# oscka/rag-llm-k8s

Measured on AMD Instinct MI355X. Metric: end-to-end RAG query p50 latency + gen tokens/sec, Llama-3.1-8B top-k=4, higher is better.
Workload: dtype bf16; 1 GPU; model=Llama-3.1-8B-Instruct, embedder=all-MiniLM-L6-v2, index=FlatL2 10000 vectors (HBM-resident; 10000 embedded chunks), retrieve_k=4, context_k=4, global_batch=32, seq_len=5198, parallelism=dp1

## Files before the change

### csrc/kernels/gemm_w4.hip

```cpp
#include <stdlib.h>

#include <utility>

#include "common.h"
using namespace ragk;

namespace {

constexpr int WBM = 256, WBN = 256, WBK = 64;
constexpr int W4_THREADS = 256;
constexpr int W_TILE_A = WBM * WBK * 2;
constexpr int W_TILE_B = WBN * WBK * 2;
constexpr int W_BUF = W_TILE_A + W_TILE_B;
constexpr int W4_LDS = 2 * W_BUF;
constexpr int WGROUP_M = 8;
constexpr int W4_MIN_KT = 3;

__device__ __forceinline__ int wswz(int row, int chunk) { return chunk ^ ((row >> 1) & 7); }

template <typename F, int... Ms>
__device__ __forceinline__ void static_for_impl(F&& f, std::integer_sequence<int, Ms...>) {
  (f(std::integral_constant<int, Ms>{}), ...);
}
template <int N, typename F>
// ... 390 lines not shown

__device__ __forceinline__ void w4_read_f0(int g, const unsigned (&rbA)[2], const unsigned (&rbB)[2],
                                           bf16x8 (&a0)[8], bf16x8 (&b0)[8]) {
  const unsigned buf = (unsigned)(g & 1) * W_BUF;
  const unsigned rb0 = rbB[0] + buf, ra0 = rbA[0] + buf;
  static_for<8>([&](auto jc) __attribute__((always_inline)) {
    constexpr int j = decltype(jc)::value;
    h_read(b0[j], rb0, j * 2048);
  });
  static_for<8>([&](auto ic) __attribute__((always_inline)) {
    constexpr int i = decltype(ic)::value;
    h_read(a0[i], ra0, i * 2048);
  });
}

__device__ __forceinline__ void w4_origin(int tile, int nwg, int tiles_m, int tiles_n, int& m0, int& n0) {
  const int logical = xcd_remap(tile, nwg);
  const int group = logical / (WGROUP_M * tiles_n);
  const int first_m = group * WGROUP_M;
  const int gm = min(tiles_m - first_m, WGROUP_M);
  const int in_group = logical % (WGROUP_M * tiles_n);
  m0 = (first_m + in_group % gm) * WBM;
  n0 = (in_group / gm) * WBN;
}

template <int EPI, bool OUT_F32, bool KSPLIT = false>
__global__ __launch_bounds__(W4_THREADS, 1) void gemm_w4_kernel(const bf16_t* __restrict__ A, int lda,
                                                                const bf16_t* __restrict__ B, int ldb, void* C,
                                                                int ldc, const bf16_t* __restrict__ bias,
                                                                const bf16_t* resid, int ldr, int M, int N, int K,
                                                                int nsplit, RopeKV rk) {
  __shared__ __attribute__((aligned(16))) char smem[W4_LDS];
  const int tid = threadIdx.x, lane = tid & 63;
  const int wid = __builtin_amdgcn_readfirstlane(tid >> 6);
  const int wr = wid >> 1, wc = wid & 1;
  const int fr = lane & 15, fh = lane >> 4;
  const int tiles_m = (M + WBM - 1) / WBM, tiles_n = (N + WBN - 1) / WBN;
  const int nwg = tiles_m * tiles_n;
  const int nwt = KSPLIT ? nwg * nsplit : nwg;
  const int nk = K / WBK;
  const int Nout = EPI == EPI_SILU_MUL ? N / 2 : N;
  const i32x4 srd_a = make_srd(A, (unsigned)M * (unsigned)lda * 2u);
  const i32x4 srd_b = make_srd(B, (unsigned)N * (unsigned)ldb * 2u);

  constexpr int EV = w4_epi_vmem<EPI, OUT_F32>();
  constexpr int VMH0 = H_VM + EV > 63 ? 63 : H_VM + EV;
  constexpr bool LATE_F0 = !(EPI == EPI_NONE || EPI == EPI_SILU_MUL || (EPI == EPI_RESID && !OUT_F32));
  static_assert(EPI != EPI_ROPE_KV || (!OUT_F32 && !KSPLIT), "rope epilogue: bf16 output, no split-K");

  int tile = blockIdx.x;
  int z = KSPLIT ? tile / nwg : 0;
  int m0, n0;
  w4_origin(tile - z * nwg, nwg, tiles_m, tiles_n, m0, n0);
  int off_a[8], off_b[8];
  w4_offsets<false>(lda, m0, M, wid, lane, off_a);
  w4_offsets<true>(ldb, n0, N, wid, lane, off_b);
  if constexpr (KSPLIT) {
#pragma unroll
    for (int i = 0; i < 8; ++i) {
      off_a[i] += z * K * 2;
      off_b[i] += z * K * 2;
    }
  }
  w4_stage(srd_a, off_a, 0, smem, wid);
  w4_stage(srd_b, off_b, 0, smem + W_TILE_A, wid);
  w4_stage(srd_a, off_a, WBK, smem + W_BUF, wid);
  w4_stage(srd_b, off_b, WBK, smem + W_BUF + W_TILE_A, wid);
  __builtin_amdgcn_s_waitcnt(0x0F70);
// ... 14 lines not shown
    }
  }

  f32x4 acc[8][8];
  int g = 0;
  for (;;) {
    const int next = tile + (int)gridDim.x;
    const bool has_next = next < nwt;
    w4_iter_h<true, VMH0>(smem, g, srd_a, srd_b, off_a, off_b, 2, wid, rbA, rbB, acc, a0, b0, a1, b1);
    ++g;
    for (int t = 1; t + 2 < nk; ++t, ++g)
      w4_iter_h<false, H_VM>(smem, g, srd_a, srd_b, off_a, off_b, t + 2, wid, rbA, rbB, acc, a0, b0, a1, b1);
    int nm0, nn0;
    const int ntile = has_next ? next : tile;
    const int nz = KSPLIT ? ntile / nwg : 0;
    w4_origin(ntile - nz * nwg, nwg, tiles_m, tiles_n, nm0, nn0);
    {
      int ln;
      asm volatile("v_mbcnt_lo_u32_b32 %0, -1, 0\n\tv_mbcnt_hi_u32_b32 %0, -1, %0" : "=v"(ln));
      w4_offsets<false>(lda, nm0, M, wid, ln, off_a);
      w4_offsets<true>(ldb, nn0, N, wid, ln, off_b);
      if constexpr (KSPLIT) {
#pragma unroll
        for (int i = 0; i < 8; ++i) {
          off_a[i] += nz * K * 2;
          off_b[i] += nz * K * 2;
        }
      }
    }
    w4_iter_h<false, H_VM>(smem, g, srd_a, srd_b, off_a, off_b, 0, wid, rbA, rbB, acc, a0, b0, a1, b1);
    ++g;
// ... 32 lines not shown
  }
}

static int g_w4_grid = -1;
static int w4_grid(int nwg) {
  if (g_w4_grid < 0) {
    int cus = 0, dev = 0;
    if (hipGetDevice(&dev) != hipSuccess ||
        hipDeviceGetAttribute(&cus, hipDeviceAttributeMultiprocessorCount, dev) != hipSuccess)
      cus = 256;
    g_w4_grid = (cus / 8) * 8;
  }
  return (g_w4_grid == 0 || g_w4_grid >= nwg) ? nwg : g_w4_grid;
}

template <int EPI, bool F32>
int launch_w4(const void* A, int lda, const void* B, int ldb, void* C, int ldc, const void* bias, const void* resid,
              int ldr, int M, int N, int K, hipStream_t st) {
  const int nwg = ((M + WBM - 1) / WBM) * ((N + WBN - 1) / WBN);
  hipLaunchKernelGGL((gemm_w4_kernel<EPI, F32>), dim3(w4_grid(nwg)), dim3(W4_THREADS), 0, st, (const bf16_t*)A, lda,
                     (const bf16_t*)B, ldb, C, ldc, (const bf16_t*)bias, (const bf16_t*)resid, ldr, M, N, K, 1,
                     RopeKV{});
  return (int)hipGetLastError();
}

}

RAGK_API int ragk_gemm_w4_set_grid(int g) {
  g_w4_grid = g < 0 ? -1 : g;
  return 0;
}

RAGK_API int ragk_gemm_w4(const void* A, int lda, const void* B, int ldb, void* C, int ldc, const void* bias,
                          const void* resid, int ldr, int M, int N, int K, int epi, int out_f32, hipStream_t st) {
  if (M <= 0 || N <= 0 || K <= 0) return 0;
  if (K % WBK != 0 || K / WBK < W4_MIN_KT) return (int)hipErrorInvalidValue;
  const long long rows_b = (epi == EPI_SILU_MUL) ? 2LL * N : (long long)N;
  if ((long long)M * lda * 2 >= (1LL << 31) || rows_b * ldb * 2 >= (1LL << 31))
    return (int)hipErrorInvalidValue;
  if (epi == EPI_SILU_MUL) {
    if (N % 128 != 0 || out_f32) return (int)hipErrorInvalidValue;
    return launch_w4<EPI_SILU_MUL, false>(A, lda, B, ldb, C, ldc, bias, resid, ldr, M, 2 * N, K, st);
  }
  if (N % 8 != 0) return (int)hipErrorInvalidValue;
#define RAGK_W4_CASE(E) \
  case E:               \
    return out_f32 ? launch_w4<E, true>(A, lda, B, ldb, C, ldc, bias, resid, ldr, M, N, K, st) \
                   : launch_w4<E, false>(A, lda, B, ldb, C, ldc, bias, resid, ldr, M, N, K, st);
  switch (epi) {
    RAGK_W4_CASE(EPI_NONE)
    RAGK_W4_CASE(EPI_BIAS)
    RAGK_W4_CASE(EPI_RESID)
    RAGK_W4_CASE(EPI_BIAS_RESID)
    RAGK_W4_CASE(EPI_BIAS_GELU)
    RAGK_W4_CASE(EPI_GELU)
    RAGK_W4_CASE(EPI_BIAS_GELU_TANH)
    default:
      return (int)hipErrorInvalidValue;
  }
#undef RAGK_W4_CASE
}

RAGK_API int ragk_gemm_w4_splitk(const void* A, int lda, const void* B, int ldb, float* P, int M, int N, int K,
                                 int nsplit, hipStream_t st) {
  if (M <= 0 || N <= 0 || K <= 0) return 0;
  if (nsplit < 1 || K % nsplit || (K / nsplit) % WBK || (K / nsplit) / WBK < W4_MIN_KT || N % 8 || !P)
    return (int)hipErrorInvalidValue;
  if ((long long)M * lda * 2 >= (1LL << 31) || (long long)N * ldb * 2 >= (1LL << 31)) return (int)hipErrorInvalidValue;
  const int nwg = ((M + WBM - 1) / WBM) * ((N + WBN - 1) / WBN);
  hipLaunchKernelGGL((gemm_w4_kernel<EPI_NONE, true, true>), dim3(w4_grid(nwg * nsplit)), dim3(W4_THREADS), 0, st,
                     (const bf16_t*)A, lda, (const bf16_t*)B, ldb, (void*)P, N, nullptr, nullptr, 0, M, N, K / nsplit,
                     nsplit, RopeKV{});
  return (int)hipGetLastError();
}

RAGK_API int ragk_gemm_w4_rope_kv(const void* A, int lda, const void* B, int ldb, void* C, int ldc, int M, int K,
                                  const int* pos, const int* slot, const float* cos_t, const float* sin_t, void* kc,
                                  void* vc, int Hq, int Hkv, int BS, hipStream_t st) {
  if (M <= 0) return 0;
  const int N = (Hq + 2 * Hkv) * 128;
  if (K % WBK != 0 || K / WBK < W4_MIN_KT || Hq < 1 || Hkv < 1 || BS < 1 || N % WBN != 0) return (int)hipErrorInvalidValue;
  if (!pos || !slot || !cos_t || !sin_t || !kc || !vc || ldc % 8 != 0) return (int)hipErrorInvalidValue;
  if ((long long)M * lda * 2 >= (1LL << 31) || (long long)N * ldb * 2 >= (1LL << 31)) return (int)hipErrorInvalidValue;
  const int nwg = ((M + WBM - 1) / WBM) * (N / WBN);
  const RopeKV rk{pos, slot, cos_t, sin_t, (bf16_t*)kc, (bf16_t*)vc, Hq, Hkv, BS};
  hipLaunchKernelGGL((gemm_w4_kernel<EPI_ROPE_KV, false>), dim3(w4_grid(nwg)), dim3(W4_THREADS), 0, st,
                     (const bf16_t*)A, lda, (const bf16_t*)B, ldb, C, ldc, nullptr, nullptr, 0, M, N, K, 1, rk);
  return (int)hipGetLastError();
}
```

### rag_llm_k8s_amd/engine/llm_engine.py

```python
from __future__ import annotations

import itertools
import logging
import os
import threading
import time
from collections import deque
from dataclasses import dataclass, field
from typing import List, Optional

import numpy as np
import torch

from ..models.llama import StepInput
from ..ops.backend import AttnMeta
from ..ops.fp8 import kv_cache_dtype_name, kv_cache_torch_dtype
from ..utils import faults
from .kv_manager import BLOCK, make_block_manager

SMALL_BATCH_TOPK_MAX_B = 64
SMALL_BATCH_TOPK_CHUNK = 4096

log = logging.getLogger(__name__)

# ... 395 lines not shown
            p = np.arange(start, start + n, dtype=np.int32)
            if start + n <= len(s.prompt):
                ids.append(s.prompt_np[start:start + n])
            else:
                ids.append(np.asarray([s.token_at(i) for i in range(start, start + n)], dtype=np.int32))
            pos.append(p)
            slots.append(table[p // BLOCK] * BLOCK + p % BLOCK)
            cu.append(cu[-1] + n)
            kvl.append(start + n)
            qlens.append(n)
            nb = min(len(table), self.max_blocks)
            bts[ci, :nb] = table[:nb]
            if start + n == len(s.prompt) or (start + n == s.length and start >= len(s.prompt)):
                out_rows.append(cu[-1] - 1)
                out_seqs.append(s)
        from ..ops.native import build_prefill_tiles

        m = self.model
        tiles = build_prefill_tiles(qlens, m.Hq, m.Hkv)
        meta = AttnMeta("prefill", self._h2d_i32(kvl), self._h2d_i32(bts), cu_q=self._h2d_i32(cu),
                        tiles=tiles.to(self.device), host_kv_lens=kvl, host_q_lens=qlens)
        ntok = cu[-1]
        inp = StepInput(self._h2d_i32(np.concatenate(ids)), self._h2d_i32(np.concatenate(pos)),
                        self._h2d_i32(np.concatenate(slots)), meta,
                        self._h2d_i32(out_rows) if out_rows else self._h2d_i32([ntok - 1]))
        return inp, out_seqs, ntok

    @staticmethod
    def _split_chunks(chunks, parts):
        total = sum(n for _, _, n in chunks)
        target = -(-total // parts)
        out, cur, room = [], [], target
        for s, start, n in chunks:
            while n > 0:
                k = min(n, room)
                cur.append((s, start, k))
                start, n, room = start + k, n - k, room - k
                if room == 0 and len(out) < parts - 1:
                    out.append(cur)
                    cur, room = [], target
# ... 346 lines not shown
```

### rag_llm_k8s_amd/models/llama.py

```python
from __future__ import annotations

import json
import math
import os
from dataclasses import dataclass, field
from typing import List, Optional

import torch

from ..ops.backend import AttnMeta, get_backend
from ..ops.fp8 import FP8, alloc_fp8_kv, check_fp8_kv_head_dim, kv_cache_torch_dtype
from ..ops.reference import pack_gate_up, rope_tables

DECODE_DOWN_SKINNY_MAX_M = 4
DECODE_OPROJ_MERGE_MAX_M = 2


@dataclass
class LlamaConfig:
    vocab_size: int = 128256
    hidden_size: int = 4096
    intermediate_size: int = 14336
    num_hidden_layers: int = 32
    num_attention_heads: int = 32
# ... 177 lines not shown
        self.dtype = "mxfp4"
        return self

    def nbytes(self):
        t = [self.embed, self.norm, self.lm_head] + [v for l in self.layers for v in l.values()]
        return sum(x.nbytes() if hasattr(x, "dequant") else x.numel() * x.element_size() for x in t)


@dataclass
class StepInput:
    ids: torch.Tensor
    positions: torch.Tensor
    slots: torch.Tensor
    meta: AttnMeta
    logits_idx: Optional[torch.Tensor] = None
    carry: Optional[torch.Tensor] = None
    carry_src: Optional[torch.Tensor] = None


class LlamaModel:
    def __init__(self, cfg: LlamaConfig, weights: LlamaWeights, device, comm=None, max_positions=None):
        self.cfg, self.w, self.device = cfg, weights, torch.device(device)
        self.be = get_backend(self.device)
        g = weights.geom()
        self.Hq, self.Hkv, self.D, self.I, self.Vl = g["Hq"], g["Hkv"], g["D"], g["I"], g["V"]
        self.comm = comm
        self.tp_rank = weights.tp_rank
        mp = max_positions or cfg.max_position_embeddings
        cos, sin = rope_tables(self.D, mp, cfg.rope_theta, cfg.rope_scaling)
        self.cos, self.sin = cos.to(self.device), sin.to(self.device)
# ... 39 lines not shown
        else:
            be.gemm(attn, L["wo"], out=h)

    def _mlp_block(self, L, h):
        be, c = self.be, self.cfg
        xn = be.rmsnorm(h, L["ln_post"], c.rms_norm_eps)
        a = be.gemm(xn, L["wgu"], epi="silu_mul")
        if self.tp_rank == 0:
            be.gemm(a, L["wdown"], resid=h, epi="resid", out=h)
        else:
            be.gemm(a, L["wdown"], out=h)

    def _final(self, h, inp: StepInput):
        if inp.logits_idx is not None:
            h = self.be.gather_rows(h, inp.logits_idx)
        return self.be.rmsnorm(h, self.w.norm, self.cfg.rms_norm_eps)

    def _tp(self):
        return self.comm is not None and self.comm.size > 1

    def _decode_part_ok(self, inp: StepInput, h):
        if inp.meta is None or inp.meta.kind != "decode" or inp.slots is None:
            return False
        L, M = self.w.layers[0], h.shape[0]
        if self._tp() and not self.comm.fused_decode_ok(M, h.shape[1]):
            return False
        return self.be.part_ok(M, L["wqkv"]) and self.be.part_ok(M, L["wo"]) and self.be.part_ok(M, L["wdown"])

    def hidden_states_decode_part(self, inp: StepInput, h):
        be, w, c = self.be, self.w, self.cfg
        Hq, Hkv, D = self.Hq, self.Hkv, self.D
# ... 40 lines not shown
        if inp.logits_idx is not None:
            xn = be.gather_rows(xn, inp.logits_idx)
        return xn

    def hidden_states(self, inp: StepInput):
        be, w = self.be, self.w
        h = be.embed(inp.ids, w.embed, carry=inp.carry, prev=inp.carry_src)
        if self._decode_part_ok(inp, h):
            return self.hidden_states_decode_part(inp, h)
        attn = torch.empty((h.shape[0], self.Hq * self.D), dtype=h.dtype, device=h.device)
        if self.comm is None and inp.meta is not None and inp.meta.kind != "decode":
            L0 = w.layers[0]
            ns = (be.prefill_nsplit(h.shape[0], L0["wo"]), be.prefill_nsplit(h.shape[0], L0["wdown"]))
            if max(ns) > 1:
                return self.hidden_states_splitk(inp, h, attn, *ns)
        for li, L in enumerate(w.layers):
            self._attn_block(li, L, h, inp, attn)
            self._allreduce(h)
            self._mlp_block(L, h)
            self._allreduce(h)
        return self._final(h, inp)

    def hidden_states_splitk(self, inp: StepInput, h, attn, ns_o, ns_d):
        be, w, c = self.be, self.w, self.cfg
        Hq, Hkv, D = self.Hq, self.Hkv, self.D
        layers = w.layers
        xn = be.rmsnorm(h, layers[0]["ln_in"], c.rms_norm_eps)
        for li, L in enumerate(layers):
            kc, vc = self.kv_cache[li]
            qkv = be.gemm_rope_kv(xn, L["wqkv"], inp.positions, self.cos, self.sin, inp.slots, kc, vc, Hq, Hkv, D)
            be.attn_prefill(qkv, kc, vc, inp.meta, attn, Hq, Hkv, D)
            if ns_o > 1:
                xn = be.add_partials_rmsnorm(be.gemm_splitk(attn, L["wo"], ns_o), h, L["ln_post"], c.rms_norm_eps)
            else:
                be.gemm(attn, L["wo"], resid=h, epi="resid", out=h)
                xn = be.rmsnorm(h, L["ln_post"], c.rms_norm_eps)
            a = be.gemm(xn, L["wgu"], epi="silu_mul")
            nxt = layers[li + 1]["ln_in"] if li + 1 < len(layers) else w.norm
            if ns_d > 1:
                xn = be.add_partials_rmsnorm(be.gemm_splitk(a, L["wdown"], ns_d), h, nxt, c.rms_norm_eps)
            else:
                be.gemm(a, L["wdown"], resid=h, epi="resid", out=h)
                xn = be.rmsnorm(h, nxt, c.rms_norm_eps)
        if inp.logits_idx is not None:
            xn = be.gather_rows(xn, inp.logits_idx)
        return xn

    def hidden_states_sp(self, inp: StepInput):
        be, w, c, comm = self.be, self.w, self.cfg, self.comm
        tp, r = comm.size, comm.rank
        Hq, Hkv, D, H = self.Hq, self.Hkv, self.D, c.hidden_size
        T = inp.ids.shape[0]
        S = -(-T // tp)
        Tp = S * tp
        ids = inp.ids
        if Tp != T:
            ids = torch.cat([ids, ids.new_zeros(Tp - T)])
# ... 52 lines not shown
```

### rag_llm_k8s_amd/ops/_lib.py

```python
from __future__ import annotations

import ctypes
import os
import threading

import torch

_HERE = os.path.dirname(os.path.abspath(__file__))
LIB_PATH = os.path.join(os.path.dirname(_HERE), "_lib", "libragk_hip.so")

P, I, F, S, U64 = ctypes.c_void_p, ctypes.c_int, ctypes.c_float, ctypes.c_void_p, ctypes.c_uint64

_SIGS = {
    "ragk_gemm": [P, I, P, I, P, I, P, P, I, I, I, I, I, I, S],
    "ragk_gemm_path": [I, P, I, P, I, P, I, P, P, I, I, I, I, I, S],
    "ragk_gemm_pp": [P, I, P, I, P, I, P, P, I, I, I, I, I, I, S],
    "ragk_gemm_w4_set_grid": [I],
    "ragk_gemm_stream_set_nt": [I],
    "ragk_gemm_stream_set_diag": [I],
    "ragk_gemm_stream_set_pair_rows": [I],
    "ragk_gemm_w4": [P, I, P, I, P, I, P, P, I, I, I, I, I, I, S],
    "ragk_gemm_w4_rope_kv": [P, I, P, I, P, I, I, I, P, P, P, P, P, P, I, I, I, S],
    "ragk_gemm_w4_splitk": [P, I, P, I, P, I, I, I, I, S],
    "ragk_gemm_part": [P, I, P, I, P, I, I, I, I, S],
    "ragk_gemm_part_norm": [P, I, P, F, P, I, P, I, I, I, I, S],
    "ragk_gemm_part_fp8": [P, I, P, I, P, P, I, I, I, I, S],
    "ragk_attn_decode_set_nt": [I],
    "ragk_attn_decode_set_nw8": [I],
    "ragk_attn_decode_set_defer": [I],
    "ragk_attn_decode_set_diag": [I],
    "ragk_attn_decode_set_kl": [I],
    "ragk_gemm_part_merge": [P, P, P, I, P, I, I, I, P, I, P, P, I, I, I, I, S],
    "ragk_gemm_part_merge_ok": [I, I, I, I, I],
    "ragk_gemm_stream_part": [P, I, P, I, P, I, I, I, I, I, S],
    "ragk_gemm_part_silu": [P, I, P, I, P, I, I, I, I, S],
    "ragk_gemm_part_silu_ok": [I, I, I, I],
    "ragk_mlp_engine_ok": [I, I, I, I],
    "ragk_mlp_engine_set_nt": [I],
# ... 151 lines not shown
```

### rag_llm_k8s_amd/ops/backend.py

```python
from __future__ import annotations

import math
from dataclasses import dataclass, field
from typing import List, Optional

import torch

from . import reference as R
from . import mxfp4
from .fp8 import Fp8KV, Fp8Weight, reference_linear
from .mxfp4 import Mxfp4Weight

KV_BLOCK = 64
_QUANT = (Fp8Weight, Mxfp4Weight)


@dataclass
class AttnMeta:
    kind: str
    kv_lens: torch.Tensor
    block_tables: torch.Tensor
    cu_q: Optional[torch.Tensor] = None
    tiles: Optional[torch.Tensor] = None
    part_tiles: int = 4
    max_parts: int = 1
    ws_o: Optional[torch.Tensor] = None
    ws_ml: Optional[torch.Tensor] = None
    host_kv_lens: List[int] = field(default_factory=list)
    host_q_lens: List[int] = field(default_factory=list)


class TorchBackend:
    name = "torch"

    def __init__(self, device="cpu"):
        self.device = torch.device(device)

    def gemm(self, x, w, bias=None, resid=None, epi="none", out=None, out_f32=False):
# ... 140 lines not shown
        out.copy_(o.reshape(T, Hq * D))
        return out

    def attn_decode_rope(self, P, positions, cos_t, sin_t, slots, kc, vc, meta: AttnMeta, out, Hq, Hkv, D,
                         defer_merge=False):
        q = torch.empty((P.shape[1], Hq * D), dtype=out.dtype, device=out.device)
        self.rope_kv_partials(P, q, positions, cos_t, sin_t, slots, kc, vc, Hq, Hkv, D)
        return self.attn_decode(q, kc, vc, meta, out, Hq, Hkv, D)

    def part_merge_ok(self, M, meta: AttnMeta, w, Hq, D):
        return False

    def prefill_nsplit(self, M, w):
        return 1

    def attn_decode(self, q, kc, vc, meta: AttnMeta, out, Hq, Hkv, D):
        B = q.shape[0]
        cu = torch.arange(B + 1, dtype=torch.int32)
        m = AttnMeta("prefill", meta.kv_lens, meta.block_tables, cu_q=cu, host_kv_lens=meta.host_kv_lens)
        return self.attn_prefill(q, kc, vc, m, out, Hq, Hkv, D)

    def attn_encoder(self, qkv, cu, lens_host, tiles, out, H, D):
        T = qkv.shape[0]
        q = qkv[:, :H * D].reshape(T, H, D)
        k = qkv[:, H * D:2 * H * D].reshape(T, H, D)
        v = qkv[:, 2 * H * D:3 * H * D].reshape(T, H, D)
        o = R.attention_varlen(q, k, v, cu.cpu(), lens_host, False, 1.0 / math.sqrt(D), cu_kv=cu.cpu())
        out.copy_(o.reshape(T, H * D))
        return out

# ... 36 lines not shown
            _, _, pick = R.sample_from_logits_candidates(v, i, t, float(top_ps[b]), u)
            out[b] = pick
        return out


class NativeBackend(TorchBackend):
    name = "native"

    def __init__(self, device="cuda"):
        super().__init__(device)
        from . import native

        self.n = native
        native._lib.lib()

    def gemm(self, x, w, bias=None, resid=None, epi="none", out=None, out_f32=False):
        if isinstance(w, Fp8Weight):
            return self.n.gemm_fp8(x, w, bias=bias, resid=resid, epi=epi, out=out, out_f32=out_f32)
        if isinstance(w, Mxfp4Weight):
            return self.n.gemm_mxfp4(x, w, bias=bias, resid=resid, epi=epi, out=out, out_f32=out_f32)
        return self.n.gemm(x, w, bias=bias, resid=resid, epi=epi, out=out, out_f32=out_f32)

    def rmsnorm(self, x, w, eps, out=None):
        return self.n.rmsnorm(x, w, eps, out=out)

    def layernorm(self, x, g, b, eps, out=None, resid=None):
        return self.n.layernorm(x, g, b, eps, out=out, resid=resid)

    def embed(self, ids, table, out=None, carry=None, prev=None):
        return self.n.embed(ids, table, out=out, carry=carry, prev=prev)

    def embed_ln(self, ids, pos_ids, word, pos, type_row, g, b, eps, do_ln=True):
        return self.n.embed_ln(ids, pos_ids, word, pos, type_row, g, b, eps, do_ln=do_ln)

    def gather_rows(self, x, idx):
        return self.n.gather_rows(x, idx)
# ... 39 lines not shown
    def add_partials_rmsnorm(self, P, h, w, eps):
        return self.n.add_partials_rmsnorm(P, h, w, eps)

    def mlp_engine_ok(self, M, w_gu, w_down):
        return self.n.mlp_engine_ok(M, w_gu, w_down)

    def mlp_engine(self, xn, w_gu, w_down, h):
        return self.n.mlp_engine(xn, w_gu, w_down, h)

    def mlp_engine_tail(self, P, h, gamma, eps, w_gu, w_down):
        return self.n.mlp_engine_tail(P, h, gamma, eps, w_gu, w_down)

    def rope_kv_partials(self, P, q_out, positions, cos_t, sin_t, slots, kc, vc, Hq, Hkv, D):
        self.n.rope_kv_partials(P, q_out, positions, cos_t, sin_t, slots, kc, vc, Hq, Hkv, D)

    def attn_prefill(self, q, kc, vc, meta: AttnMeta, out, Hq, Hkv, D):
        return self.n.attn_prefill(q, kc, vc, meta.cu_q, meta.kv_lens, meta.tiles, out, Hq, Hkv, D, causal=True,
                                   paged=True, block_tables=meta.block_tables)

    def attn_decode_rope(self, P, positions, cos_t, sin_t, slots, kc, vc, meta: AttnMeta, out, Hq, Hkv, D,
                         defer_merge=False):
        return self.n.attn_decode_rope(P, positions, cos_t, sin_t, slots, kc, vc, meta.block_tables, meta.kv_lens, out,
                                       Hq, Hkv, D, meta.part_tiles, meta.max_parts, meta.ws_o, meta.ws_ml,
                                       defer_merge=defer_merge)

    def prefill_nsplit(self, M, w):
        if isinstance(w, _QUANT):
            return 1
        return self.n.prefill_nsplit(M, w.shape[0], w.shape[1])

    def gemm_splitk(self, x, w, nsplit):
        return self.n.gemm_splitk(x, w, nsplit)

    def part_merge_ok(self, M, meta: AttnMeta, w, Hq, D):
        return (self.enable_part and D == 128 and not isinstance(w, Mxfp4Weight)
                and self.n.gemm_part_merge_ok(M, w, Hq, meta.max_parts, meta.ws_o))

    def gemm_part_merge(self, attn_out, meta: AttnMeta, w, Hq):
        return self.n.gemm_part_merge(attn_out, meta.kv_lens, meta.part_tiles, meta.max_parts, meta.ws_o, meta.ws_ml,
                                      Hq, w)

    def attn_decode(self, q, kc, vc, meta: AttnMeta, out, Hq, Hkv, D):
        return self.n.attn_decode(q, kc, vc, meta.block_tables, meta.kv_lens, out, Hq, Hkv, D, meta.part_tiles,
                                  meta.max_parts, meta.ws_o, meta.ws_ml)

    def attn_encoder(self, qkv, cu, lens_host, tiles, out, H, D):
        return self.n.attn_prefill(qkv, qkv[:, H * D:], qkv[:, 2 * H * D:], cu, _lens_dev(cu), tiles, out, H, H, D,
# ... 34 lines not shown
```

### rag_llm_k8s_amd/ops/native.py

```python
from __future__ import annotations

import math
import os
import threading

import torch

from . import _lib
from ._lib import check, ptr, stream_ptr
from .fp8 import FP8, Fp8KV
from .reference import EPI


def _req(cond, msg):
    if not cond:
        raise ValueError(msg)


def _kv8(k_cache, v_cache, Hkv, D, dev):
    _req(isinstance(k_cache, Fp8KV) and isinstance(v_cache, Fp8KV), "fp8 KV cache: both k and v must be Fp8KV")
    _req(D == 128, "fp8 KV cache needs head_dim 128")
    kd = k_cache.data
    _req(kd.dim() == 4 and kd.shape[1] == Hkv and kd.shape[2] == 64 and kd.shape[3] == D, "fp8 cache [nb,Hkv,64,128]")
    for side, c in (("k", k_cache), ("v", v_cache)):
# ... 107 lines not shown
    check(_lib.lib().ragk_gemm_w4_rope_kv(x.data_ptr(), x.stride(0), w.data_ptr(), w.stride(0), out.data_ptr(),
                                          out.stride(0), M, K, positions.data_ptr(), slots.data_ptr(),
                                          cos_t.data_ptr(), sin_t.data_ptr(), k_cache.data_ptr(), v_cache.data_ptr(),
                                          Hq, Hkv, k_cache.shape[2], stream_ptr()), "ragk_gemm_w4_rope_kv")
    return out


def _gemm_blas(x, w, resid, out, epi):
    if epi == "resid":
        if out.data_ptr() == resid.data_ptr() and out.stride() == resid.stride():
            return out.addmm_(x, w.t())
        return torch.addmm(resid, x, w.t(), out=out)
    return torch.mm(x, w.t(), out=out)


def gemm(x, w, bias=None, resid=None, epi="none", out=None, out_f32=False, path=None):
    _bf16_2d(x, "x")
    _bf16_2d(w, "w")
    M, K = x.shape
    e = EPI[epi]
    N = w.shape[0] // 2 if epi == "silu_mul" else w.shape[0]
    _req(w.shape[1] == K, "K mismatch %s vs %s" % (tuple(x.shape), tuple(w.shape)))
    _req(K % 128 == 0, "K must be a multiple of 128 (got %d)" % K)
    if epi == "silu_mul":
        _req(N % 64 == 0, "silu_mul needs N % 64 == 0")
    if "bias" in epi:
        _req(bias is not None and bias.is_cuda and bias.dtype == torch.bfloat16 and bias.numel() == N
             and bias.is_contiguous(), "bias must be bf16[N]")
    if "resid" in epi:
        _bf16_2d(resid, "resid")
        _req(resid.shape == (M, N), "resid shape")
    odt = torch.float32 if out_f32 else torch.bfloat16
    if out is None:
        out = torch.empty((M, N), dtype=odt, device=x.device)
    _req(out.dtype == odt and out.shape == (M, N) and out.stride(1) == 1, "out shape/dtype")
    if M > 64 and N % 8 != 0 and epi != "silu_mul":
        raise ValueError("tile GEMM needs N % 8 == 0")
    if M == 0:
        return out
    _al16(x, "x")
    _al16(w, "w")
    L = _lib.lib()
    ldr = resid.stride(0) if resid is not None else 0
    if (path is None and PREFILL_BLAS != "none" and not out_f32 and bias is None and use_pp(M, N, K, epi)
            and ((epi == "none" and PREFILL_BLAS in ("plain", "all"))
                 or (epi == "resid" and PREFILL_BLAS in ("resid", "all")))):
        return _gemm_blas(x, w, resid, out, epi)
    if path is None and use_pp(M, N, K, epi):
        rows = w.shape[0]
        fits = x.stride(0) * M * 2 < 2 ** 31 and w.stride(0) * rows * 2 < 2 ** 31
        path = 6 if fits else 2
    if path is None and STREAM_DEFAULT and use_stream(M, N, K, epi):
        path = 5
    if path is None and DEC_DEFAULT and use_dec(M, N, K, epi):
        path = 4
    _req(path in (None, 0, 1, 2, 3, 4, 5, 6), "unknown GEMM path %r" % (path,))
    if path in (0, 2, 6) or (path is None and M > 64):
        _al16(out, "out")
# ... 5 lines not shown
        rc = _gemm_stream(x, w, None, out, bias, resid, ldr, M, N, K, epi, e, out_f32)
    elif path == 4:
        ws, cnt = dec_workspace(x.device)
        S = L.ragk_gemm_dec_splits(N, K, e)
        need = S * (2 if epi == "silu_mul" else 1) * M * N
        _req(S == 1 or need <= ws.numel(), "decode GEMM workspace too small (%d > %d floats)" % (need, ws.numel()))
        _req(-(-N // 128) <= cnt.numel(), "too many n-tiles for the counter buffer")
        rc = L.ragk_gemm_dec(x.data_ptr(), x.stride(0), w.data_ptr(), w.stride(0), out.data_ptr(), out.stride(0),
                             ptr(bias), ptr(resid), ldr, M, N, K, e, int(out_f32), S, ws.data_ptr(), cnt.data_ptr(),
                             stream_ptr())
    elif path == 2:
        rc = L.ragk_gemm_pp(x.data_ptr(), x.stride(0), w.data_ptr(), w.stride(0), out.data_ptr(), out.stride(0),
                            ptr(bias), ptr(resid), ldr, M, N, K, e, int(out_f32), stream_ptr())
    elif path == 6:
        rc = L.ragk_gemm_w4(x.data_ptr(), x.stride(0), w.data_ptr(), w.stride(0), out.data_ptr(), out.stride(0),
                            ptr(bias), ptr(resid), ldr, M, N, K, e, int(out_f32), stream_ptr())
    elif path is None:
        rc = L.ragk_gemm(x.data_ptr(), x.stride(0), w.data_ptr(), w.stride(0), out.data_ptr(), out.stride(0),
                         ptr(bias), ptr(resid), ldr, M, N, K, e, int(out_f32), stream_ptr())
    else:
        rc = L.ragk_gemm_path(path, x.data_ptr(), x.stride(0), w.data_ptr(), w.stride(0), out.data_ptr(),
                              out.stride(0), ptr(bias), ptr(resid), ldr, M, N, K, e, stream_ptr())
    check(rc, "ragk_gemm")
    return out


PART_MIN_BLOCKS = 512
_part_cfg = [False]


def gemm_part_slabs(M, N, K, ks=None):
# ... 126 lines not shown
    if not PREFILL_SPLITK or M < PREFILL_SPLITK_MIN_M:
        return 1
    cus = _cu_count()
    tiles = -(-M // 256) * -(-N // 256)
    best, best_s = 0.0, 1
    for s in (1, 2):
        if K % (64 * s) or K // s < 4 * 64:
            continue
        wt = tiles * s
        eff = wt / (-(-wt // cus) * cus) - 0.02 * (s - 1)
        if eff > best + 1e-9:
            best, best_s = eff, s
    return best_s


def gemm_splitk(x, w, nsplit, out=None):
    _bf16_2d(x, "x")
    _bf16_2d(w, "w")
    M, K = x.shape
    N = w.shape[0]
    _req(w.shape[1] == K and K % (64 * nsplit) == 0 and K // nsplit >= 256 and N % 8 == 0, "gemm_splitk shape")
    if out is None:
        out = torch.empty((nsplit, M, N), dtype=torch.float32, device=x.device)
    _req(out.dtype == torch.float32 and out.is_contiguous() and out.numel() >= nsplit * M * N
         and out.data_ptr() % 16 == 0, "gemm_splitk out: contiguous fp32 slabs, 16-byte aligned")
    _al16(x, "x")
    _al16(w, "w")
    check(_lib.lib().ragk_gemm_w4_splitk(x.data_ptr(), x.stride(0), w.data_ptr(), w.stride(0), out.data_ptr(), M, N, K,
                                         nsplit, stream_ptr()), "ragk_gemm_w4_splitk")
    return out


def gemm_part_merge_ok(M, w, Hq, max_parts, ws_o):
    from .fp8 import Fp8Weight

    if ws_o is None or max_parts < 2:
        return False
    wt = w.w8 if isinstance(w, Fp8Weight) else w
    N, K = wt.shape
    ks, S = gemm_part_slabs(M, N, K)
    return S > 0 and bool(_lib.lib().ragk_gemm_part_merge_ok(M, K, Hq, max_parts, ks))


def gemm_part_merge(attn_out, kv_lens, part_tiles, max_parts, ws_o, ws_ml, Hq, w, out=None):
# ... 575 lines not shown


def build_prefill_tiles(q_lens, Hq, Hkv):
    import numpy as np

    qt = prefill_qtile(Hq, Hkv)
    ql = np.asarray(q_lens, dtype=np.int64)
    nt = (ql + qt - 1) // qt
    seq = np.repeat(np.arange(len(ql)), nt)
    first = np.repeat(np.cumsum(nt) - nt, nt)
    q0 = (np.arange(int(nt.sum())) - first) * qt
    order = np.argsort(-q0, kind="stable")
    return torch.from_numpy(np.stack([seq[order], q0[order]], 1).astype(np.int32)).reshape(-1, 2)


def attn_prefill(q, k, v, cu_q, kv_lens, tiles, out, Hq, Hkv, D, causal=True, paged=True, block_tables=None,
                 cu_kv=None, kv_stride=0, scale=None):
    _req(q.dtype == torch.bfloat16 and q.stride(-1) == 1, "q")
    _req(tiles.dtype == torch.int32 and tiles.is_cuda and tiles.is_contiguous(), "tiles int32 on GPU")
    _req(D in (32, 64, 128), "head_dim must be 32/64/128")
    if isinstance(k, Fp8KV) or isinstance(v, Fp8KV):
        _req(paged and causal, "fp8 KV cache: paged causal attention only")
        _kv8(k, v, Hkv, D, q.device)
        _req(block_tables is not None and block_tables.dtype == torch.int32, "block_tables int32")
        _req(block_tables.stride(0) <= 2048, "prefill block tables wider than 2048 blocks (128k tokens)")
        scale = 1.0 / math.sqrt(D) if scale is None else scale
        check(_lib.lib().ragk_attn_prefill_fp8(
            q.data_ptr(), q.stride(0), k.data.data_ptr(), v.data.data_ptr(), k.scale.data_ptr(), v.scale.data_ptr(),
            block_tables.data_ptr(), block_tables.stride(0), cu_q.data_ptr(), kv_lens.data_ptr(), tiles.data_ptr(),
            tiles.shape[0], out.data_ptr(), out.stride(0), Hq, Hkv, D, float(scale), stream_ptr()),
# ... 325 lines not shown
```

Measured before the change: 1682 generated tokens/s (aggregate over all GPUs).

## Restrict last-layer prefill attention and MLP GEMMs to tiles holding logit rows

In the final transformer layer during prefill, only the rows whose logits are sampled need the attention output, o-proj, and MLP. The change builds a list of 256-row M tiles and attention query tiles that contain those rows, and passes the M-tile list into the gemm_w4 kernel (including split-K) so only those tiles are computed. K/V are still written for all tokens via the full QKV GEMM. This removes roughly one layer's worth of non-KV prefill compute, at the cost of extra host-side list building, H2D copies and new kernel template variants.

```diff
diff --git a/csrc/kernels/gemm_w4.hip b/csrc/kernels/gemm_w4.hip
--- a/csrc/kernels/gemm_w4.hip
+++ b/csrc/kernels/gemm_w4.hip
@@ -428,28 +428,34 @@
   });
 }
 
-__device__ __forceinline__ void w4_origin(int tile, int nwg, int tiles_m, int tiles_n, int& m0, int& n0) {
+template <bool MT = false>
+__device__ __forceinline__ void w4_origin(int tile, int nwg, int tiles_m, int tiles_n, int& m0, int& n0,
+                                          const int* __restrict__ mt = nullptr, int mt_max = 0) {
   const int logical = xcd_remap(tile, nwg);
   const int group = logical / (WGROUP_M * tiles_n);
   const int first_m = group * WGROUP_M;
   const int gm = min(tiles_m - first_m, WGROUP_M);
   const int in_group = logical % (WGROUP_M * tiles_n);
-  m0 = (first_m + in_group % gm) * WBM;
+  int mi = first_m + in_group % gm;
+  if constexpr (MT) mi = (int)min((unsigned)mt[__builtin_amdgcn_readfirstlane(mi)], (unsigned)mt_max);
+  m0 = mi * WBM;
   n0 = (in_group / gm) * WBN;
 }
 
-template <int EPI, bool OUT_F32, bool KSPLIT = false>
+template <int EPI, bool OUT_F32, bool KSPLIT = false, bool MT = false>
 __global__ __launch_bounds__(W4_THREADS, 1) void gemm_w4_kernel(const bf16_t* __restrict__ A, int lda,
                                                                 const bf16_t* __restrict__ B, int ldb, void* C,
                                                                 int ldc, const bf16_t* __restrict__ bias,
                                                                 const bf16_t* resid, int ldr, int M, int N, int K,
-                                                                int nsplit, RopeKV rk) {
+                                                                int nsplit, RopeKV rk,
+                                                                const int* __restrict__ m_tiles, int n_m_tiles) {
   __shared__ __attribute__((aligned(16))) char smem[W4_LDS];
   const int tid = threadIdx.x, lane = tid & 63;
   const int wid = __builtin_amdgcn_readfirstlane(tid >> 6);
   const int wr = wid >> 1, wc = wid & 1;
   const int fr = lane & 15, fh = lane >> 4;
-  const int tiles_m = (M + WBM - 1) / WBM, tiles_n = (N + WBN - 1) / WBN;
+  const int tiles_m = MT ? n_m_tiles : (M + WBM - 1) / WBM, tiles_n = (N + WBN - 1) / WBN;
+  const int mt_max = (M + WBM - 1) / WBM - 1;
   const int nwg = tiles_m * tiles_n;
   const int nwt = KSPLIT ? nwg * nsplit : nwg;
   const int nk = K / WBK;
@@ -461,11 +467,13 @@
   constexpr int VMH0 = H_VM + EV > 63 ? 63 : H_VM + EV;
   constexpr bool LATE_F0 = !(EPI == EPI_NONE || EPI == EPI_SILU_MUL || (EPI == EPI_RESID && !OUT_F32));
   static_assert(EPI != EPI_ROPE_KV || (!OUT_F32 && !KSPLIT), "rope epilogue: bf16 output, no split-K");
+  static_assert(!MT || EPI == EPI_NONE || ((EPI == EPI_RESID || EPI == EPI_SILU_MUL) && !OUT_F32 && !KSPLIT),
+                "M-tile list: none / residual / SiLU*up epilogues and the split-K slabs");
 
   int tile = blockIdx.x;
   int z = KSPLIT ? tile / nwg : 0;
   int m0, n0;
-  w4_origin(tile - z * nwg, nwg, tiles_m, tiles_n, m0, n0);
+  w4_origin<MT>(tile - z * nwg, nwg, tiles_m, tiles_n, m0, n0, m_tiles, mt_max);
   int off_a[8], off_b[8];
   w4_offsets<false>(lda, m0, M, wid, lane, off_a);
   w4_offsets<true>(ldb, n0, N, wid, lane, off_b);
@@ -510,7 +518,7 @@
     int nm0, nn0;
     const int ntile = has_next ? next : tile;
     const int nz = KSPLIT ? ntile / nwg : 0;
-    w4_origin(ntile - nz * nwg, nwg, tiles_m, tiles_n, nm0, nn0);
+    w4_origin<MT>(ntile - nz * nwg, nwg, tiles_m, tiles_n, nm0, nn0, m_tiles, mt_max);
     {
       int ln;
       asm volatile("v_mbcnt_lo_u32_b32 %0, -1, 0\n\tv_mbcnt_hi_u32_b32 %0, -1, %0" : "=v"(ln));
@@ -573,14 +581,31 @@
   return (g_w4_grid == 0 || g_w4_grid >= nwg) ? nwg : g_w4_grid;
 }
 
+constexpr bool w4_mt_epi(int e) { return e == EPI_NONE || e == EPI_RESID || e == EPI_SILU_MUL; }
+
 template <int EPI, bool F32>
 int launch_w4(const void* A, int lda, const void* B, int ldb, void* C, int ldc, const void* bias, const void* resid,
-              int ldr, int M, int N, int K, hipStream_t st) {
-  const int nwg = ((M + WBM - 1) / WBM) * ((N + WBN - 1) / WBN);
+              int ldr, int M, int N, int K, const int* m_tiles, int n_m_tiles, hipStream_t st) {
+  const int tiles_n = (N + WBN - 1) / WBN;
+  if (m_tiles) {
+    if constexpr (w4_mt_epi(EPI) && !F32) {
+      hipLaunchKernelGGL((gemm_w4_kernel<EPI, F32, false, true>), dim3(w4_grid(n_m_tiles * tiles_n)),
+                         dim3(W4_THREADS), 0, st, (const bf16_t*)A, lda, (const bf16_t*)B, ldb, C, ldc,
+                         (const bf16_t*)bias, (const bf16_t*)resid, ldr, M, N, K, 1, RopeKV{}, m_tiles, n_m_tiles);
+      return (int)hipGetLastError();
+    } else {
+      return (int)hipErrorInvalidValue;
+    }
+  }
+  const int nwg = ((M + WBM - 1) / WBM) * tiles_n;
   hipLaunchKernelGGL((gemm_w4_kernel<EPI, F32>), dim3(w4_grid(nwg)), dim3(W4_THREADS), 0, st, (const bf16_t*)A, lda,
                      (const bf16_t*)B, ldb, C, ldc, (const bf16_t*)bias, (const bf16_t*)resid, ldr, M, N, K, 1,
-                     RopeKV{});
+                     RopeKV{}, nullptr, 0);
   return (int)hipGetLastError();
+}
+
+static bool w4_mt_ok(const int* m_tiles, int n_m_tiles, int M) {
+  return !m_tiles || (n_m_tiles >= 1 && n_m_tiles <= (M + WBM - 1) / WBM);
 }
 
 }
@@ -591,21 +616,24 @@
 }
 
 RAGK_API int ragk_gemm_w4(const void* A, int lda, const void* B, int ldb, void* C, int ldc, const void* bias,
-                          const void* resid, int ldr, int M, int N, int K, int epi, int out_f32, hipStream_t st) {
-  if (M <= 0 || N <= 0 || K <= 0) return 0;
+                          const void* resid, int ldr, int M, int N, int K, int epi, int out_f32, const int* m_tiles,
+                          int n_m_tiles, hipStream_t st) {
+  if (M <= 0 || N <= 0 || K <= 0 || (m_tiles && n_m_tiles == 0)) return 0;
+  if (!w4_mt_ok(m_tiles, n_m_tiles, M)) return (int)hipErrorInvalidValue;
   if (K % WBK != 0 || K / WBK < W4_MIN_KT) return (int)hipErrorInvalidValue;
   const long long rows_b = (epi == EPI_SILU_MUL) ? 2LL * N : (long long)N;
   if ((long long)M * lda * 2 >= (1LL << 31) || rows_b * ldb * 2 >= (1LL << 31))
     return (int)hipErrorInvalidValue;
   if (epi == EPI_SILU_MUL) {
     if (N % 128 != 0 || out_f32) return (int)hipErrorInvalidValue;
-    return launch_w4<EPI_SILU_MUL, false>(A, lda, B, ldb, C, ldc, bias, resid, ldr, M, 2 * N, K, st);
+    return launch_w4<EPI_SILU_MUL, false>(A, lda, B, ldb, C, ldc, bias, resid, ldr, M, 2 * N, K, m_tiles, n_m_tiles,
+                                          st);
   }
   if (N % 8 != 0) return (int)hipErrorInvalidValue;
 #define RAGK_W4_CASE(E) \
   case E:               \
-    return out_f32 ? launch_w4<E, true>(A, lda, B, ldb, C, ldc, bias, resid, ldr, M, N, K, st) \
-                   : launch_w4<E, false>(A, lda, B, ldb, C, ldc, bias, resid, ldr, M, N, K, st);
+    return out_f32 ? launch_w4<E, true>(A, lda, B, ldb, C, ldc, bias, resid, ldr, M, N, K, m_tiles, n_m_tiles, st) \
+                   : launch_w4<E, false>(A, lda, B, ldb, C, ldc, bias, resid, ldr, M, N, K, m_tiles, n_m_tiles, st);
   switch (epi) {
     RAGK_W4_CASE(EPI_NONE)
     RAGK_W4_CASE(EPI_BIAS)
@@ -621,15 +649,23 @@
 }
 
 RAGK_API int ragk_gemm_w4_splitk(const void* A, int lda, const void* B, int ldb, float* P, int M, int N, int K,
-                                 int nsplit, hipStream_t st) {
-  if (M <= 0 || N <= 0 || K <= 0) return 0;
+                                 int nsplit, const int* m_tiles, int n_m_tiles, hipStream_t st) {
+  if (M <= 0 || N <= 0 || K <= 0 || (m_tiles && n_m_tiles == 0)) return 0;
+  if (!w4_mt_ok(m_tiles, n_m_tiles, M)) return (int)hipErrorInvalidValue;
   if (nsplit < 1 || K % nsplit || (K / nsplit) % WBK || (K / nsplit) / WBK < W4_MIN_KT || N % 8 || !P)
     return (int)hipErrorInvalidValue;
   if ((long long)M * lda * 2 >= (1LL << 31) || (long long)N * ldb * 2 >= (1LL << 31)) return (int)hipErrorInvalidValue;
+  if (m_tiles) {
+    const int nwt = n_m_tiles * ((N + WBN - 1) / WBN) * nsplit;
+    hipLaunchKernelGGL((gemm_w4_kernel<EPI_NONE, true, true, true>), dim3(w4_grid(nwt)), dim3(W4_THREADS), 0, st,
+                       (const bf16_t*)A, lda, (const bf16_t*)B, ldb, (void*)P, N, nullptr, nullptr, 0, M, N,
+                       K / nsplit, nsplit, RopeKV{}, m_tiles, n_m_tiles);
+    return (int)hipGetLastError();
+  }
   const int nwg = ((M + WBM - 1) / WBM) * ((N + WBN - 1) / WBN);
   hipLaunchKernelGGL((gemm_w4_kernel<EPI_NONE, true, true>), dim3(w4_grid(nwg * nsplit)), dim3(W4_THREADS), 0, st,
                      (const bf16_t*)A, lda, (const bf16_t*)B, ldb, (void*)P, N, nullptr, nullptr, 0, M, N, K / nsplit,
-                     nsplit, RopeKV{});
+                     nsplit, RopeKV{}, nullptr, 0);
   return (int)hipGetLastError();
 }
 
@@ -644,6 +680,6 @@
   const int nwg = ((M + WBM - 1) / WBM) * (N / WBN);
   const RopeKV rk{pos, slot, cos_t, sin_t, (bf16_t*)kc, (bf16_t*)vc, Hq, Hkv, BS};
   hipLaunchKernelGGL((gemm_w4_kernel<EPI_ROPE_KV, false>), dim3(w4_grid(nwg)), dim3(W4_THREADS), 0, st,
-                     (const bf16_t*)A, lda, (const bf16_t*)B, ldb, C, ldc, nullptr, nullptr, 0, M, N, K, 1, rk);
+                     (const bf16_t*)A, lda, (const bf16_t*)B, ldb, C, ldc, nullptr, nullptr, 0, M, N, K, 1, rk, nullptr, 0);
   return (int)hipGetLastError();
 }
diff --git a/rag_llm_k8s_amd/engine/llm_engine.py b/rag_llm_k8s_amd/engine/llm_engine.py
--- a/rag_llm_k8s_amd/engine/llm_engine.py
+++ b/rag_llm_k8s_amd/engine/llm_engine.py
@@ -433,16 +433,22 @@
             if start + n == len(s.prompt) or (start + n == s.length and start >= len(s.prompt)):
                 out_rows.append(cu[-1] - 1)
                 out_seqs.append(s)
-        from ..ops.native import build_prefill_tiles
+        from ..ops.native import build_last_rows_lists, build_prefill_tiles
 
         m = self.model
         tiles = build_prefill_tiles(qlens, m.Hq, m.Hkv)
         meta = AttnMeta("prefill", self._h2d_i32(kvl), self._h2d_i32(bts), cu_q=self._h2d_i32(cu),
                         tiles=tiles.to(self.device), host_kv_lens=kvl, host_q_lens=qlens)
         ntok = cu[-1]
+        cuts = getattr(m, "prefill_last_rows_enabled", None)
+        cuts = self.tp_size == 1 and cuts is not None and cuts()
+        m_tiles = None
+        if cuts and out_rows:
+            tl, mt = build_last_rows_lists(qlens, out_rows, m.Hq, m.Hkv, tiles=tiles)
+            meta.tiles_last, m_tiles = self._h2d_i32(tl.numpy()), self._h2d_i32(mt.numpy())
         inp = StepInput(self._h2d_i32(np.concatenate(ids)), self._h2d_i32(np.concatenate(pos)),
                         self._h2d_i32(np.concatenate(slots)), meta,
-                        self._h2d_i32(out_rows) if out_rows else self._h2d_i32([ntok - 1]))
+                        self._h2d_i32(out_rows if out_rows or cuts else [ntok - 1]), m_tiles=m_tiles)
         return inp, out_seqs, ntok
 
     @staticmethod
diff --git a/rag_llm_k8s_amd/models/llama.py b/rag_llm_k8s_amd/models/llama.py
--- a/rag_llm_k8s_amd/models/llama.py
+++ b/rag_llm_k8s_amd/models/llama.py
@@ -215,6 +215,7 @@
     slots: torch.Tensor
     meta: AttnMeta
     logits_idx: Optional[torch.Tensor] = None
+    m_tiles: Optional[torch.Tensor] = None
     carry: Optional[torch.Tensor] = None
     carry_src: Optional[torch.Tensor] = None
 
@@ -284,7 +285,27 @@
     def _final(self, h, inp: StepInput):
         if inp.logits_idx is not None:
             h = self.be.gather_rows(h, inp.logits_idx)
+            if h.shape[0] == 0:
+                return h
         return self.be.rmsnorm(h, self.w.norm, self.cfg.rms_norm_eps)
+
+    @staticmethod
+    def prefill_last_rows_enabled():
+        return os.environ.get("RAGK_PREFILL_LAST_ROWS", "1") != "0"
+
+    def _last_rows(self, inp: StepInput, M):
+        if (self.comm is not None or inp.meta is None or inp.meta.kind == "decode" or inp.logits_idx is None
+                or not self.prefill_last_rows_enabled()):
+            return None
+        if inp.logits_idx.numel() == 0:
+            return "skip"
+        if inp.m_tiles is None or inp.meta.tiles_last is None:
+            return None
+        L, be = self.w.layers[-1], self.be
+        if not (be.m_tiles_ok(M, L["wo"], "resid") and be.m_tiles_ok(M, L["wgu"], "silu_mul")
+                and be.m_tiles_ok(M, L["wdown"], "resid")):
+            return None
+        return "tiles"
 
     def _tp(self):
         return self.comm is not None and self.comm.size > 1
@@ -355,33 +376,59 @@
             ns = (be.prefill_nsplit(h.shape[0], L0["wo"]), be.prefill_nsplit(h.shape[0], L0["wdown"]))
             if max(ns) > 1:
                 return self.hidden_states_splitk(inp, h, attn, *ns)
+        last = self._last_rows(inp, h.shape[0])
         for li, L in enumerate(w.layers):
+            if last is not None and li + 1 == len(w.layers):
+                self._last_layer_rows(li, L, h, inp, attn, last)
+                break
             self._attn_block(li, L, h, inp, attn)
             self._allreduce(h)
             self._mlp_block(L, h)
             self._allreduce(h)
         return self._final(h, inp)
 
+    def _last_layer_rows(self, li, L, h, inp: StepInput, attn, mode):
+        be, c = self.be, self.cfg
+        Hq, Hkv, D = self.Hq, self.Hkv, self.D
+        kc, vc = self.kv_cache[li]
+        xn = be.rmsnorm(h, L["ln_in"], c.rms_norm_eps)
+        qkv = be.gemm_rope_kv(xn, L["wqkv"], inp.positions, self.cos, self.sin, inp.slots, kc, vc, Hq, Hkv, D)
+        if mode == "skip":
+            return
+        mt = inp.m_tiles
+        be.attn_prefill(qkv, kc, vc, inp.meta, attn, Hq, Hkv, D, tiles=inp.meta.tiles_last)
+        be.gemm(attn, L["wo"], resid=h, epi="resid", out=h, m_tiles=mt)
+        xn = be.rmsnorm(h, L["ln_post"], c.rms_norm_eps)
+        a = be.gemm(xn, L["wgu"], epi="silu_mul", m_tiles=mt)
+        be.gemm(a, L["wdown"], resid=h, epi="resid", out=h, m_tiles=mt)
+
     def hidden_states_splitk(self, inp: StepInput, h, attn, ns_o, ns_d):
         be, w, c = self.be, self.w, self.cfg
         Hq, Hkv, D = self.Hq, self.Hkv, self.D
         layers = w.layers
+        last = self._last_rows(inp, h.shape[0])
         xn = be.rmsnorm(h, layers[0]["ln_in"], c.rms_norm_eps)
         for li, L in enumerate(layers):
             kc, vc = self.kv_cache[li]
+            cut = last if li + 1 == len(layers) else None
+            rows = {"m_tiles": inp.m_tiles} if cut == "tiles" else {}
+            blocks = {"tiles": inp.meta.tiles_last} if cut == "tiles" else {}
             qkv = be.gemm_rope_kv(xn, L["wqkv"], inp.positions, self.cos, self.sin, inp.slots, kc, vc, Hq, Hkv, D)
-            be.attn_prefill(qkv, kc, vc, inp.meta, attn, Hq, Hkv, D)
+            if cut == "skip":
+                return h.new_empty((0, h.shape[1]))
+            be.attn_prefill(qkv, kc, vc, inp.meta, attn, Hq, Hkv, D, **blocks)
             if ns_o > 1:
-                xn = be.add_partials_rmsnorm(be.gemm_splitk(attn, L["wo"], ns_o), h, L["ln_post"], c.rms_norm_eps)
+                xn = be.add_partials_rmsnorm(be.gemm_splitk(attn, L["wo"], ns_o, **rows), h, L["ln_post"],
+                                             c.rms_norm_eps)
             else:
-                be.gemm(attn, L["wo"], resid=h, epi="resid", out=h)
+                be.gemm(attn, L["wo"], resid=h, epi="resid", out=h, **rows)
                 xn = be.rmsnorm(h, L["ln_post"], c.rms_norm_eps)
-            a = be.gemm(xn, L["wgu"], epi="silu_mul")
+            a = be.gemm(xn, L["wgu"], epi="silu_mul", **rows)
             nxt = layers[li + 1]["ln_in"] if li + 1 < len(layers) else w.norm
             if ns_d > 1:
-                xn = be.add_partials_rmsnorm(be.gemm_splitk(a, L["wdown"], ns_d), h, nxt, c.rms_norm_eps)
+                xn = be.add_partials_rmsnorm(be.gemm_splitk(a, L["wdown"], ns_d, **rows), h, nxt, c.rms_norm_eps)
             else:
-                be.gemm(a, L["wdown"], resid=h, epi="resid", out=h)
+                be.gemm(a, L["wdown"], resid=h, epi="resid", out=h, **rows)
                 xn = be.rmsnorm(h, nxt, c.rms_norm_eps)
         if inp.logits_idx is not None:
             xn = be.gather_rows(xn, inp.logits_idx)
diff --git a/rag_llm_k8s_amd/ops/_lib.py b/rag_llm_k8s_amd/ops/_lib.py
--- a/rag_llm_k8s_amd/ops/_lib.py
+++ b/rag_llm_k8s_amd/ops/_lib.py
@@ -19,9 +19,9 @@
     "ragk_gemm_stream_set_nt": [I],
     "ragk_gemm_stream_set_diag": [I],
     "ragk_gemm_stream_set_pair_rows": [I],
-    "ragk_gemm_w4": [P, I, P, I, P, I, P, P, I, I, I, I, I, I, S],
+    "ragk_gemm_w4": [P, I, P, I, P, I, P, P, I, I, I, I, I, I, P, I, S],
     "ragk_gemm_w4_rope_kv": [P, I, P, I, P, I, I, I, P, P, P, P, P, P, I, I, I, S],
-    "ragk_gemm_w4_splitk": [P, I, P, I, P, I, I, I, I, S],
+    "ragk_gemm_w4_splitk": [P, I, P, I, P, I, I, I, I, P, I, S],
     "ragk_gemm_part": [P, I, P, I, P, I, I, I, I, S],
     "ragk_gemm_part_norm": [P, I, P, F, P, I, P, I, I, I, I, S],
     "ragk_gemm_part_fp8": [P, I, P, I, P, P, I, I, I, I, S],
diff --git a/rag_llm_k8s_amd/ops/backend.py b/rag_llm_k8s_amd/ops/backend.py
--- a/rag_llm_k8s_amd/ops/backend.py
+++ b/rag_llm_k8s_amd/ops/backend.py
@@ -22,6 +22,7 @@
     block_tables: torch.Tensor
     cu_q: Optional[torch.Tensor] = None
     tiles: Optional[torch.Tensor] = None
+    tiles_last: Optional[torch.Tensor] = None
     part_tiles: int = 4
     max_parts: int = 1
     ws_o: Optional[torch.Tensor] = None
@@ -192,6 +193,9 @@
     def prefill_nsplit(self, M, w):
         return 1
 
+    def m_tiles_ok(self, M, w, epi="none"):
+        return False
+
     def attn_decode(self, q, kc, vc, meta: AttnMeta, out, Hq, Hkv, D):
         B = q.shape[0]
         cu = torch.arange(B + 1, dtype=torch.int32)
@@ -258,12 +262,20 @@
         self.n = native
         native._lib.lib()
 
-    def gemm(self, x, w, bias=None, resid=None, epi="none", out=None, out_f32=False):
+    def gemm(self, x, w, bias=None, resid=None, epi="none", out=None, out_f32=False, m_tiles=None):
+        if m_tiles is not None and isinstance(w, _QUANT):
+            raise ValueError("m_tiles: bf16 weights only")
         if isinstance(w, Fp8Weight):
             return self.n.gemm_fp8(x, w, bias=bias, resid=resid, epi=epi, out=out, out_f32=out_f32)
         if isinstance(w, Mxfp4Weight):
             return self.n.gemm_mxfp4(x, w, bias=bias, resid=resid, epi=epi, out=out, out_f32=out_f32)
-        return self.n.gemm(x, w, bias=bias, resid=resid, epi=epi, out=out, out_f32=out_f32)
+        return self.n.gemm(x, w, bias=bias, resid=resid, epi=epi, out=out, out_f32=out_f32, m_tiles=m_tiles)
+
+    def m_tiles_ok(self, M, w, epi="none"):
+        if isinstance(w, _QUANT):
+            return False
+        N = w.shape[0] // 2 if epi == "silu_mul" else w.shape[0]
+        return self.n.gemm_m_tiles_ok(M, N, w.shape[1], epi, ldb=w.stride(0))
 
     def rmsnorm(self, x, w, eps, out=None):
         return self.n.rmsnorm(x, w, eps, out=out)
@@ -333,9 +345,9 @@
     def rope_kv_partials(self, P, q_out, positions, cos_t, sin_t, slots, kc, vc, Hq, Hkv, D):
         self.n.rope_kv_partials(P, q_out, positions, cos_t, sin_t, slots, kc, vc, Hq, Hkv, D)
 
-    def attn_prefill(self, q, kc, vc, meta: AttnMeta, out, Hq, Hkv, D):
-        return self.n.attn_prefill(q, kc, vc, meta.cu_q, meta.kv_lens, meta.tiles, out, Hq, Hkv, D, causal=True,
-                                   paged=True, block_tables=meta.block_tables)
+    def attn_prefill(self, q, kc, vc, meta: AttnMeta, out, Hq, Hkv, D, tiles=None):
+        return self.n.attn_prefill(q, kc, vc, meta.cu_q, meta.kv_lens, meta.tiles if tiles is None else tiles, out,
+                                   Hq, Hkv, D, causal=True, paged=True, block_tables=meta.block_tables)
 
     def attn_decode_rope(self, P, positions, cos_t, sin_t, slots, kc, vc, meta: AttnMeta, out, Hq, Hkv, D,
                          defer_merge=False):
@@ -348,8 +360,8 @@
             return 1
         return self.n.prefill_nsplit(M, w.shape[0], w.shape[1])
 
-    def gemm_splitk(self, x, w, nsplit):
-        return self.n.gemm_splitk(x, w, nsplit)
+    def gemm_splitk(self, x, w, nsplit, m_tiles=None):
+        return self.n.gemm_splitk(x, w, nsplit, m_tiles=m_tiles)
 
     def part_merge_ok(self, M, meta: AttnMeta, w, Hq, D):
         return (self.enable_part and D == 128 and not isinstance(w, Mxfp4Weight)
diff --git a/rag_llm_k8s_amd/ops/native.py b/rag_llm_k8s_amd/ops/native.py
--- a/rag_llm_k8s_amd/ops/native.py
+++ b/rag_llm_k8s_amd/ops/native.py
@@ -145,7 +145,21 @@
     return torch.mm(x, w.t(), out=out)
 
 
-def gemm(x, w, bias=None, resid=None, epi="none", out=None, out_f32=False, path=None):
+def _m_tiles_arg(m_tiles, M, dev):
+    _req(isinstance(m_tiles, torch.Tensor) and m_tiles.dtype == torch.int32 and m_tiles.dim() == 1
+         and m_tiles.is_contiguous() and m_tiles.is_cuda and m_tiles.device == dev, "m_tiles: int32 [n] on the GPU")
+    _req(m_tiles.numel() <= -(-M // 256), "m_tiles: more entries than 256-row tiles")
+    return m_tiles.data_ptr(), m_tiles.numel()
+
+
+def gemm_m_tiles_ok(M, N, K, epi="none", lda=None, ldb=None):
+    if epi not in ("none", "resid", "silu_mul") or PREFILL_BLAS != "none" or not use_pp(M, N, K, epi):
+        return False
+    rows = 2 * N if epi == "silu_mul" else N
+    return (lda or K) * M * 2 < 2 ** 31 and (ldb or K) * rows * 2 < 2 ** 31
+
+
+def gemm(x, w, bias=None, resid=None, epi="none", out=None, out_f32=False, path=None, m_tiles=None):
     _bf16_2d(x, "x")
     _bf16_2d(w, "w")
     M, K = x.shape
@@ -173,6 +187,16 @@
     _al16(w, "w")
     L = _lib.lib()
     ldr = resid.stride(0) if resid is not None else 0
+    mt_ptr, mt_n = None, 0
+    if m_tiles is not None:
+        _req(path in (None, 6), "m_tiles: only the gemm_w4 path takes an M-tile list")
+        _req(epi in ("none", "resid", "silu_mul") and not out_f32, "m_tiles: epi none / resid / silu_mul, bf16 out")
+        _req(K % 64 == 0 and K >= 192 and (N % 128 == 0 if epi == "silu_mul" else N % 8 == 0), "m_tiles: gemm_w4 shape")
+        _req(x.stride(0) * M * 2 < 2 ** 31 and w.stride(0) * w.shape[0] * 2 < 2 ** 31, "m_tiles: operand past 2 GiB")
+        mt_ptr, mt_n = _m_tiles_arg(m_tiles, M, x.device)
+        if mt_n == 0:
+            return out
+        path = 6
     if (path is None and PREFILL_BLAS != "none" and not out_f32 and bias is None and use_pp(M, N, K, epi)
             and ((epi == "none" and PREFILL_BLAS in ("plain", "all"))
                  or (epi == "resid" and PREFILL_BLAS in ("resid", "all")))):
@@ -208,7 +232,7 @@
                             ptr(bias), ptr(resid), ldr, M, N, K, e, int(out_f32), stream_ptr())
     elif path == 6:
         rc = L.ragk_gemm_w4(x.data_ptr(), x.stride(0), w.data_ptr(), w.stride(0), out.data_ptr(), out.stride(0),
-                            ptr(bias), ptr(resid), ldr, M, N, K, e, int(out_f32), stream_ptr())
+                            ptr(bias), ptr(resid), ldr, M, N, K, e, int(out_f32), mt_ptr, mt_n, stream_ptr())
     elif path is None:
         rc = L.ragk_gemm(x.data_ptr(), x.stride(0), w.data_ptr(), w.stride(0), out.data_ptr(), out.stride(0),
                          ptr(bias), ptr(resid), ldr, M, N, K, e, int(out_f32), stream_ptr())
@@ -365,7 +389,7 @@
     return best_s
 
 
-def gemm_splitk(x, w, nsplit, out=None):
+def gemm_splitk(x, w, nsplit, out=None, m_tiles=None):
     _bf16_2d(x, "x")
     _bf16_2d(w, "w")
     M, K = x.shape
@@ -377,8 +401,11 @@
          and out.data_ptr() % 16 == 0, "gemm_splitk out: contiguous fp32 slabs, 16-byte aligned")
     _al16(x, "x")
     _al16(w, "w")
+    mt_ptr, mt_n = _m_tiles_arg(m_tiles, M, x.device) if m_tiles is not None else (None, 0)
+    if m_tiles is not None and mt_n == 0:
+        return out
     check(_lib.lib().ragk_gemm_w4_splitk(x.data_ptr(), x.stride(0), w.data_ptr(), w.stride(0), out.data_ptr(), M, N, K,
-                                         nsplit, stream_ptr()), "ragk_gemm_w4_splitk")
+                                         nsplit, mt_ptr, mt_n, stream_ptr()), "ragk_gemm_w4_splitk")
     return out
 
 
@@ -984,6 +1011,29 @@
     return torch.from_numpy(np.stack([seq[order], q0[order]], 1).astype(np.int32)).reshape(-1, 2)
 
 
+M_TILE_ROWS = 256
+
+
+def build_last_rows_lists(q_lens, rows, Hq, Hkv, tiles=None):
+    import numpy as np
+
+    qt = prefill_qtile(Hq, Hkv)
+    if tiles is None:
+        tiles = build_prefill_tiles(q_lens, Hq, Hkv)
+    t = tiles.numpy().reshape(-1, 2).astype(np.int64)
+    ql = np.asarray(q_lens, dtype=np.int64)
+    cu = np.concatenate([[0], np.cumsum(ql)])
+    r = np.unique(np.asarray(rows, dtype=np.int64).reshape(-1))
+    if r.size and (r[0] < 0 or r[-1] >= cu[-1]):
+        raise ValueError("build_last_rows_lists: row outside the packed step")
+    lo = cu[t[:, 0]] + t[:, 1]
+    hi = np.minimum(lo + qt, cu[t[:, 0] + 1])
+    keep = np.searchsorted(r, lo, side="left") < np.searchsorted(r, hi, side="left")
+    tiles_last = torch.from_numpy(np.ascontiguousarray(t[keep]).astype(np.int32)).reshape(-1, 2)
+    m_tiles = torch.from_numpy(np.unique(r // M_TILE_ROWS).astype(np.int32))
+    return tiles_last, m_tiles
+
+
 def attn_prefill(q, k, v, cu_q, kv_lens, tiles, out, Hq, Hkv, D, causal=True, paged=True, block_tables=None,
                  cu_kv=None, kv_stride=0, scale=None):
     _req(q.dtype == torch.bfloat16 and q.stride(-1) == 1, "q")
```

After: 1707 generated tokens/s (aggregate over all GPUs) (median of 6 runs). 1.5% higher.
